# astojanov/Clover

Measured on AMD Instinct MI355X. Metric: int4 GEMV (CloverMatrix4::mvm) effective GB/s, algorithmic operand bytes / time, higher is better.
Workload: dtype int4; 1 GPU; CloverMatrix4::mvm 65536x65536 int4 (65536x65536 per GPU; preset c3: BASELINE configs[2] per GPU), x and result CloverVector4, STOCHASTIC_ROUNDING_DISABLED, bit-exact reference order; rows_per_gpu=65536, cols=65536, parallelism=row-shard x1, settle_launches=168

## Files before the change

clover_amd/csrc/matrix4.hip:

```cpp
#include "rng_device.h"

#include <stdlib.h>
#include <string.h>


#define MVM_CHUNK 65536u

template <int U, bool NT>
__device__ __forceinline__ void mvm_steps(const u32x4 *__restrict__ Ap, const u32x4 *xs, const float *cs, int q,
                                          uint32_t t0, float &a0, float &a1, float &a2, float &a3)
{
    u32x4 a[U];
#pragma unroll
    for (int u = 0; u < U; u++) a[u] = NT ? __builtin_nontemporal_load(&Ap[4 * (t0 + u) + q]) : Ap[4 * (t0 + u) + q];
#pragma unroll
    for (int u = 0; u < U; u++) {
        const u32x4 xv = xs[4 * (t0 + u) + q];
        const float c = cs[2 * (t0 + u) + (q >> 1)];
        a0 = __builtin_fmaf(c, (float)sdot8(a[u].x, xv.x, 0), a0);
        a1 = __builtin_fmaf(c, (float)sdot8(a[u].y, xv.y, 0), a1);
        a2 = __builtin_fmaf(c, (float)sdot8(a[u].z, xv.z, 0), a2);
        a3 = __builtin_fmaf(c, (float)sdot8(a[u].w, xv.w, 0), a3);
    }
}

template <int U, bool NT>
__device__ __forceinline__ void mvm_steps8(const u32x2 *__restrict__ Ap, const u32x2 *xs, const float *cs, int e, uint32_t t0, float &a0,
                                           float &a1)
{
    u32x2 a[U];
#pragma unroll
    for (int u = 0; u < U; u++) a[u] = NT ? __builtin_nontemporal_load(&Ap[8 * (t0 + u) + e]) : Ap[8 * (t0 + u) + e];
#pragma unroll
    for (int u = 0; u < U; u++) {
        const u32x2 xv = xs[8 * (t0 + u) + e];
        const float c = cs[2 * (t0 + u) + (e >> 2)];
        a0 = __builtin_fmaf(c, (float)sdot8(a[u].x, xv.x, 0), a0);
        a1 = __builtin_fmaf(c, (float)sdot8(a[u].y, xv.y, 0), a1);
    }
}

__device__ __forceinline__ int requantize_wave(float d, float noise, uint32_t *r_words, float *sr, float *scale)
{
    const int lane = threadIdx.x & 63;
    float m = wave_max(__builtin_fabsf(d));
    m = fix_zero_max(m);
    const float k = 7.0f / m;
    const int qv = quant1(d, k, noise);
    if (r_words) {
        uint32_t w = ((uint32_t)qv & 0xFu) << nib_shift(lane & 7);
        w |= __shfl_xor(w, 1);
        w |= __shfl_xor(w, 2);
        w |= __shfl_xor(w, 4);
        if ((lane & 7) == 0) r_words[lane >> 3] = w;
        if (lane == 0) *sr = m;
    }
    *scale = m;
    return qv;
}

struct MvmFuse {
    const uint32_t *qu;
    const float *su;
    float a;
    uint32_t *r2;
    float *sr2;
};

template <int U, bool NT, bool ST, bool FUSE, int L = 4>
__global__ __launch_bounds__(64 * L) void k_m4_mvm64(const uint8_t *__restrict__ A, const float *__restrict__ sA,
                                                  uint64_t cols, const uint8_t *__restrict__ x, const float *__restrict__ sx,
                                                  float *__restrict__ d_out, uint32_t *r, float *sr,
                                                  uint64_t *rng_state, uint64_t seq, const uint64_t *__restrict__ pow_rows, MvmFuse fuse)
{
    extern __shared__ __attribute__((aligned(16))) char smem[];
    u32x4 *xs = reinterpret_cast<u32x4 *>(smem);
    float *cs = reinterpret_cast<float *>(smem + MVM_CHUNK / 2);
    float *dsh = cs + MVM_CHUNK / 64;
    uint64_t *rbase = reinterpret_cast<uint64_t *>(dsh + 64);
    uint64_t *raw = rbase + 4;
    uint64_t *rbase2 = raw + 8, *raw2 = rbase2 + 4;
    if (ST) {
        const uint64_t a0 = rng_workgroup_begin(rng_state, seq, pow_rows, blockIdx.x, 1, (FUSE ? 4ull : 2ull) * gridDim.x, rbase);
        if (FUSE) {
            const uint64_t b2 = wave_pow_apply(pow_rows, a0, (uint64_t)gridDim.x + blockIdx.x, 1);
            if ((threadIdx.x & 63) == 0) rbase2[threadIdx.x >> 6] = b2;
        }
    }
    uint32_t fuse_w = 0;
    float fuse_s = 0.0f;
    if (FUSE && threadIdx.x < 64) {
        fuse_w = fuse.qu[blockIdx.x * 8 + (threadIdx.x >> 3)];
        fuse_s = fuse.su[blockIdx.x];
    }

    static_assert(L == 4 || (L == 8 && !ST), "the stochastic epilogue assumes 4 waves");
    constexpr int THREADS = 64 * L;
    const uint64_t rb = blockIdx.x;
    const int tid = threadIdx.x;
    const int q = tid & (L - 1);
    const int rho = tid / L;
    const uint64_t row = rb * 64 + rho;
    const u32x4 *Arow = reinterpret_cast<const u32x4 *>(A + row * (cols / 2));
    const float *sArow = sA + rb * (cols / 64);

    float a0 = 0.0f, a1 = 0.0f, a2 = 0.0f, a3 = 0.0f;

    for (uint64_t c0 = 0; c0 < cols; c0 += MVM_CHUNK) {
        const uint32_t cw = (uint32_t)((cols - c0) < MVM_CHUNK ? (cols - c0) : MVM_CHUNK);
        if (c0) __syncthreads();
        const u32x4 *xg = reinterpret_cast<const u32x4 *>(x + c0 / 2);
        {
            constexpr int NX = MVM_CHUNK / 32 / THREADS;
            constexpr int NC = MVM_CHUNK / 64 / THREADS;
            u32x4 xr[NX];
            float sa[NC], sv[NC];
            const uint32_t nx = cw / 32, nc = cw / 64;
#pragma unroll
            for (int k = 0; k < NX; k++) { const uint32_t i = tid + THREADS * k; xr[k] = xg[i < nx ? i : 0]; }
#pragma unroll
            for (int k = 0; k < NC; k++) {
                const uint32_t i = tid + THREADS * k, ii = i < nc ? i : 0;
                sa[k] = sArow[c0 / 64 + ii];
                sv[k] = sx[c0 / 64 + ii];
            }
#pragma unroll
            for (int k = 0; k < NX; k++) { const uint32_t i = tid + THREADS * k; if (i < nx) xs[i] = xr[k]; }
#pragma unroll
            for (int k = 0; k < NC; k++) { const uint32_t i = tid + THREADS * k; if (i < nc) cs[i] = (sa[k] * CLV_RCP49) * sv[k]; }
        }
        __syncthreads();

        const u32x4 *Ap = Arow + c0 / 32;
        const uint32_t npairs = cw / 128;
        uint32_t t = 0;
        if constexpr (L == 4) {
            for (; t + U <= npairs; t += U) mvm_steps<U, NT>(Ap, xs, cs, q, t, a0, a1, a2, a3);
            for (; t < npairs; t++) mvm_steps<1, NT>(Ap, xs, cs, q, t, a0, a1, a2, a3);
        } else {
            const u32x2 *Ap8 = reinterpret_cast<const u32x2 *>(Ap);
            const u32x2 *xs8 = reinterpret_cast<const u32x2 *>(xs);
            for (; t + U <= npairs; t += U) mvm_steps8<U, NT>(Ap8, xs8, cs, q, t, a0, a1);
            for (; t < npairs; t++) mvm_steps8<1, NT>(Ap8, xs8, cs, q, t, a0, a1);
        }
    }

    const float v0 = a0 + __shfl_xor(a0, 2);
    const float v1 = a1 + __shfl_xor(a1, 2);
    const float v2 = a2 + __shfl_xor(a2, 2);
    const float v3 = a3 + __shfl_xor(a3, 2);
    const float x0 = v0 + __shfl_xor(v0, 1);
    const float x1 = v1 + __shfl_xor(v1, 1);
    const float x2 = v2 + __shfl_xor(v2, 1);
    const float x3 = v3 + __shfl_xor(v3, 1);
    float dot = (x0 + x2) + (x1 + x3);
    if constexpr (L == 8) {
        const float u0 = a0 + __shfl_xor(a0, 4), u1 = a1 + __shfl_xor(a1, 4);
        const float y0 = u0 + __shfl_xor(u0, 2), y1 = u1 + __shfl_xor(u1, 2);
        const float z0 = y0 + __shfl_xor(y0, 1), z1 = y1 + __shfl_xor(y1, 1);
        dot = z0 + z1;
    }

    if (q == 0) {
        dsh[rho] = dot;
        if (d_out) d_out[row] = dot;
    }
    if (ST && tid < 4) {
        gen_blocks(rbase[tid], 1, raw, tid);
        if (FUSE) gen_blocks(rbase2[tid], 1, raw2, tid);
    }
    __syncthreads();
    if ((r || FUSE) && tid < 64) {
        float noise = 0.0f;
        if (ST) {
            const int grp = tid & 7, j = tid >> 3;
            noise = noise_of(reinterpret_cast<const uint32_t *>(raw + (size_t)(grp >> 2) * 4)[j], grp & 3);
        }
        float m;
        const int qv = requantize_wave(dsh[tid], noise, r ? r + rb * 8 : nullptr, r ? sr + rb : nullptr, &m);
        if (FUSE) {
            const float su7 = div7(fuse_s), sv7 = div7(m * fuse.a);
            const float val = __builtin_fmaf((float)qv, sv7, (float)unpack1(fuse_w, tid & 7) * su7);
            float noise2 = 0.0f;
            if (ST) {
                const int g = (tid & 7) ^ 1, j = tid >> 3;
                noise2 = noise_of(reinterpret_cast<const uint32_t *>(raw2 + (size_t)(g >> 2) * 4)[j], g & 3);
            }
            float m2;
            requantize_wave(val, noise2, fuse.r2 + rb * 8, fuse.sr2 + rb, &m2);
        }
    }
}

__global__ __launch_bounds__(256) void k_m4_quantize_strip(const float *__restrict__ A, uint64_t cols, uint32_t *__restrict__ q,
                                                           float *__restrict__ s, uint32_t strips_x, uint32_t tiles_x)
{
    __shared__ float sh[4][4];
    const uint32_t sj = blockIdx.x % strips_x;
    const uint64_t bi = blockIdx.x / strips_x;
    const int wave = threadIdx.x >> 6, lane = threadIdx.x & 63;
    const uint64_t col = (uint64_t)sj * 256 + 4 * lane;
    const bool live = col < cols;
    const uint64_t row0 = bi * 64 + wave * 16;

    f32x4 v[16];
    float m = 0.0f;
#pragma unroll
    for (int r = 0; r < 16; r++) {
        v[r] = live ? __builtin_nontemporal_load(reinterpret_cast<const f32x4 *>(A + (row0 + r) * cols + col)) : f32x4{0.0f, 0.0f, 0.0f, 0.0f};
        m = fmaxf(m, fmaxf(fmaxf(__builtin_fabsf(v[r].x), __builtin_fabsf(v[r].y)), fmaxf(__builtin_fabsf(v[r].z), __builtin_fabsf(v[r].w))));
    }
    m = row16_max(m);
    if ((lane & 15) == 0) sh[wave][lane >> 4] = m;
    __syncthreads();
    const int t = lane >> 4;
    m = fix_zero_max(fmaxf(fmaxf(sh[0][t], sh[1][t]), fmaxf(sh[2][t], sh[3][t])));
    const float k = 7.0f / m;
    if (wave == 0 && (lane & 15) == 0 && live) s[bi * tiles_x + sj * 4 + t] = m;
    const int odd = lane & 1;
#pragma unroll
    for (int r = 0; r < 16; r += 2) {
        const uint32_t h0 = quant_pack4(v[r], k), h1 = quant_pack4(v[r + 1], k);
        const uint32_t give = odd ? h0 : h1;
        const uint32_t recv = (uint32_t)__builtin_amdgcn_update_dpp(0, (int)give, 0xB1, 0xF, 0xF, false);
        const uint32_t word = odd ? (recv | (h1 << 16)) : (h0 | (recv << 16));
        if (live) __builtin_nontemporal_store(word, &q[((row0 + r + odd) * cols + (col & ~7ull)) / 8]);
    }
}

__global__ __launch_bounds__(256) void k_m4_gemm_simple(const uint8_t *__restrict__ A, const float *__restrict__ sA, uint64_t M,
                                                        uint64_t K, const uint8_t *__restrict__ B, const float *__restrict__ sB,
                                                        uint64_t N, float *__restrict__ C)
{
    const uint64_t j = (uint64_t)blockIdx.x * 16 + (threadIdx.x & 15);
    const uint64_t i = (uint64_t)blockIdx.y * 16 + (threadIdx.x >> 4);
    if (i >= M || j >= N) return;
    const uint64_t kb = K / 64;
    const u32x4 *a = reinterpret_cast<const u32x4 *>(A + i * (K / 2));
    const u32x4 *b = reinterpret_cast<const u32x4 *>(B + j * (K / 2));
    const float *sa = sA + (i >> 6) * kb;
    const float *sb = sB + (j >> 6) * kb;
    float acc = 0.0f;
    for (uint64_t blk = 0; blk < kb; blk++) {
        const int S = dot32(a[2 * blk], b[2 * blk]) + dot32(a[2 * blk + 1], b[2 * blk + 1]);
        const float c = (sa[blk] * CLV_RCP49) * sb[blk];
        acc = __builtin_fmaf(c, (float)S, acc);
    }
    C[i * N + j] = acc;
}

template <bool NT>
__global__ __launch_bounds__(256) void k_m4_restore(const uint32_t *__restrict__ q, const float *__restrict__ s, f32x4 *__restrict__ A,
                                                    uint64_t nquads, uint64_t cols)
{
    const uint64_t f0 = ((uint64_t)blockIdx.x * 4 + (threadIdx.x >> 6)) * 256;
    const int lane = threadIdx.x & 63;
    const uint64_t tiles_x = cols / 64;
    uint32_t wd[4];
    float sc[4];
#pragma unroll
    for (int j = 0; j < 4; j++) {
        const uint64_t f = f0 + 64 * j + lane, fc = f < nquads ? f : 0;
        const uint64_t e = fc * 4, row = e / cols, col = e - row * cols;
        wd[j] = q[fc >> 1];
        sc[j] = s[(row >> 6) * tiles_x + (col >> 6)];
    }
#pragma unroll
    for (int j = 0; j < 4; j++) {
        const uint64_t f = f0 + 64 * j + lane;
        const uint32_t hw = wd[j] >> (16 * (lane & 1));
        const float k = div7(sc[j]);
        f32x4 v;
        v.x = (float)(((int)(hw << 24)) >> 28) * k;
        v.y = (float)(((int)(hw << 28)) >> 28) * k;
        v.z = (float)(((int)(hw << 16)) >> 28) * k;
        v.w = (float)(((int)(hw << 20)) >> 28) * k;
        if (f < nquads) {
            if (NT) __builtin_nontemporal_store(v, &A[f]);
            else A[f] = v;
        }
    }
}

int clm4_quantize_stochastic(const float *A, uint64_t rows, uint64_t cols, int8_t *q, float *s, uint64_t *rng, hipStream_t st);
int clm4_gemm_mfma(const int8_t *A, const float *sA, uint64_t M, uint64_t K, const int8_t *B, const float *sB, uint64_t N, float *C, hipStream_t st);
int clm4_gemm_fp6(const int8_t *A, const float *sA, uint64_t M, uint64_t K, const int8_t *B, const float *sB, uint64_t N, float *C, hipStream_t st);

#define MVM_LDS_BYTES (MVM_CHUNK / 2 + (MVM_CHUNK / 64) * sizeof(float) + 64 * sizeof(float) + 256)

static int launch_mvm(const int8_t *A, const float *sA, uint64_t rows, uint64_t cols, const int8_t *x, const float *sx,
                      float *d, int8_t *r, float *sr, uint64_t *rng, hipStream_t st, const MvmFuse *fuse = nullptr)
{
    const size_t lds = MVM_LDS_BYTES;
    const dim3 grid((unsigned)(rows / 64)), block(256);
    RngTables T = {nullptr, nullptr, nullptr};
    uint64_t seq = 0;
    if (rng) {
        int rc = clv_rng_tables(&T);
        if (rc) return rc;
        seq = clv_rng_seq_for(rng, st);
    }
    const MvmFuse no_fuse = {nullptr, nullptr, 0.0f, nullptr, nullptr};
#define MVM_LAUNCH_F(NT, ST, FUSE)                                                                                               \
    hipLaunchKernelGGL((k_m4_mvm64<8, NT, ST, FUSE>), grid, block, lds, st, (const uint8_t *)A, sA, cols, (const uint8_t *)x, sx, d, \
                       (uint32_t *)r, sr, rng, seq, T.pow_rows, FUSE ? *fuse : no_fuse)
#define MVM_LAUNCH(NT, ST)                                  \
    do {                                                    \
        if (fuse) MVM_LAUNCH_F(NT, ST, true);               \
        else MVM_LAUNCH_F(NT, ST, false);                   \
    } while (0)
    const bool streaming = rows * (cols / 2) > (256ull << 20);
    const bool wide = streaming && !rng && rows / 64 <= 2ull * (uint64_t)clv_cu_count();
    if (wide) {
        if (fuse)
            hipLaunchKernelGGL((k_m4_mvm64<16, true, false, true, 8>), grid, dim3(512), lds, st, (const uint8_t *)A, sA, cols,
                               (const uint8_t *)x, sx, d, (uint32_t *)r, sr, rng, seq, T.pow_rows, *fuse);
        else
            hipLaunchKernelGGL((k_m4_mvm64<16, true, false, false, 8>), grid, dim3(512), lds, st, (const uint8_t *)A, sA, cols,
                               (const uint8_t *)x, sx, d, (uint32_t *)r, sr, rng, seq, T.pow_rows, no_fuse);
    } else if (streaming) {
        if (rng) MVM_LAUNCH(true, true); else MVM_LAUNCH(true, false);
    } else {
        if (rng) MVM_LAUNCH(false, true); else MVM_LAUNCH(false, false);
    }
#undef MVM_LAUNCH
#undef MVM_LAUNCH_F
    CLV_LAUNCH_CHECK();
    return CLV_OK;
}

#ifdef CLV_EXPERIMENTS
__global__ __launch_bounds__(256) void k_read_bw(const u32x4 *__restrict__ p, uint64_t n16, uint32_t *__restrict__ out, int nt)
{
    const uint64_t stride = (uint64_t)gridDim.x * blockDim.x;
    uint32_t acc = 0;
    uint64_t i = (uint64_t)blockIdx.x * blockDim.x + threadIdx.x;
    for (; i + 7 * stride < n16; i += 8 * stride) {
        u32x4 v[8];
#pragma unroll
        for (int u = 0; u < 8; u++) v[u] = nt ? __builtin_nontemporal_load(&p[i + u * stride]) : p[i + u * stride];
#pragma unroll
        for (int u = 0; u < 8; u++) acc ^= v[u].x ^ v[u].y ^ v[u].z ^ v[u].w;
    }
    for (; i < n16; i += stride) { const u32x4 v = p[i]; acc ^= v.x ^ v.y ^ v.z ^ v.w; }
    if (acc == 0x12345678u) out[0] = acc;
}

extern "C" int clvx_read_bw(const void *p, uint64_t bytes, int nt, int blocks_per_cu, void *out, void *stream)
{
    hipLaunchKernelGGL(k_read_bw, dim3(clv_cu_count() * blocks_per_cu), dim3(256), 0, as_stream(stream), (const u32x4 *)p, bytes / 16,
                       (uint32_t *)out, nt);
    CLV_LAUNCH_CHECK();
    return CLV_OK;
}

extern "C" int clvx_mvm_variant(int variant, const int8_t *A, const float *sA, uint64_t rows, uint64_t cols, const int8_t *x,
                                const float *sx, int8_t *r, float *sr, void *stream)
{
    const size_t lds = MVM_LDS_BYTES;
    hipStream_t st = as_stream(stream);
    const dim3 grid((unsigned)(rows / 64)), block(256);
#define CLVX_LAUNCH(U, NT)                                                                                                      \
    hipLaunchKernelGGL((k_m4_mvm64<U, NT, false, false>), grid, block, lds, st, (const uint8_t *)A, sA, cols, (const uint8_t *)x, sx, \
                       (float *)nullptr, (uint32_t *)r, sr, (uint64_t *)nullptr, 0ull, (const uint64_t *)nullptr,                      \
                       MvmFuse{nullptr, nullptr, 0.0f, nullptr, nullptr})
    switch (variant) {
    case 0: CLVX_LAUNCH(8, true); break;
    case 1: CLVX_LAUNCH(8, false); break;
    case 2: CLVX_LAUNCH(4, true); break;
    case 3: CLVX_LAUNCH(16, true); break;
    case 4: CLVX_LAUNCH(2, true); break;
    case 5: CLVX_LAUNCH(16, false); break;
    case 6: CLVX_LAUNCH(32, false); break;
#define CLVX_LAUNCH8(U, NT)                                                                                                       \
    hipLaunchKernelGGL((k_m4_mvm64<U, NT, false, false, 8>), grid, dim3(512), lds, st, (const uint8_t *)A, sA, cols, (const uint8_t *)x, \
                       sx, (float *)nullptr, (uint32_t *)r, sr, (uint64_t *)nullptr, 0ull, (const uint64_t *)nullptr,                 \
                       MvmFuse{nullptr, nullptr, 0.0f, nullptr, nullptr})
    case 7: CLVX_LAUNCH8(8, false); break;
    case 8: CLVX_LAUNCH8(16, false); break;
    case 9: CLVX_LAUNCH8(8, true); break;
    case 10: CLVX_LAUNCH8(16, true); break;
#undef CLVX_LAUNCH8
    default: clv_set_error("clvx_mvm_variant: unknown variant %d", variant); return CLV_ERR_INVALID;
    }
#undef CLVX_LAUNCH
    CLV_LAUNCH_CHECK();
    return CLV_OK;
}
#endif

static int check_mvm_args(const char *fn, const void *A, const void *sA, uint64_t rows, uint64_t cols, const void *x, const void *sx)
{
    CLV_REQUIRE(A && sA && x && sx, "%s: null pointer", fn);
    CLV_REQUIRE(rows % 64 == 0 && cols % 128 == 0, "%s: rows=%llu must be a multiple of 64 and cols=%llu of 128", fn,
                (unsigned long long)rows, (unsigned long long)cols);
    CLV_REQUIRE(rows / 64 <= 0x7FFFFFFFull, "%s: too many rows", fn);
    return CLV_OK;
}

extern "C" int clm4_restore(const int8_t *q, const float *s, uint64_t rows, uint64_t cols, float *A, void *stream)
{
    CLV_REQUIRE(A && q && s, "clm4_restore: null pointer");
    CLV_REQUIRE(rows % 128 == 0 && cols % 128 == 0, "clm4_restore: rows=%llu cols=%llu must be multiples of 128", (unsigned long long)rows,
                (unsigned long long)cols);
    if (!rows || !cols) return CLV_OK;
    const uint64_t nquads = rows * cols / 4, waves = (nquads + 255) / 256;
    CLV_REQUIRE((waves + 3) / 4 <= 0x7FFFFFFFull, "clm4_restore: matrix too large");
    if (rows * cols * sizeof(float) > (256ull << 20))
        hipLaunchKernelGGL(k_m4_restore<true>, dim3((unsigned)((waves + 3) / 4)), dim3(256), 0, as_stream(stream), (const uint32_t *)q, s,
                           (f32x4 *)A, nquads, cols);
    else
        hipLaunchKernelGGL(k_m4_restore<false>, dim3((unsigned)((waves + 3) / 4)), dim3(256), 0, as_stream(stream), (const uint32_t *)q, s,
                           (f32x4 *)A, nquads, cols);
    CLV_LAUNCH_CHECK();
    return CLV_OK;
}

extern "C" int clm4_mvm(const int8_t *A, const float *sA, uint64_t rows, uint64_t cols, const int8_t *x, const float *sx,
                        int8_t *r, float *sr, uint64_t *rng_state_dev, void *stream)
{
    int rc = check_mvm_args("clm4_mvm", A, sA, rows, cols, x, sx);
    if (rc) return rc;
    CLV_REQUIRE(r && sr, "clm4_mvm: null result pointer");
    if (!rows) return CLV_OK;
    hipStream_t st = as_stream(stream);
    return launch_mvm(A, sA, rows, cols, x, sx, nullptr, r, sr, rng_state_dev, st);
}

extern "C" int clm4_mvm_scale_and_add(const int8_t *A, const float *sA, uint64_t rows, uint64_t cols, const int8_t *x, const float *sx,
                                      const int8_t *qu, const float *su, float a, int8_t *t, float *st_, int8_t *r, float *sr,
                                      uint64_t *rng_state_dev, void *stream)
{
    int rc = check_mvm_args("clm4_mvm_scale_and_add", A, sA, rows, cols, x, sx);
    if (rc) return rc;
    CLV_REQUIRE(qu && su && r && sr, "clm4_mvm_scale_and_add: null pointer");
    CLV_REQUIRE((t == nullptr) == (st_ == nullptr), "clm4_mvm_scale_and_add: t and st must both be given or both be NULL");
    CLV_REQUIRE((const void *)r != (const void *)x && (const void *)sr != (const void *)sx,
                "clm4_mvm_scale_and_add: the result must not alias the vector being multiplied");
    if (!rows) return CLV_OK;
    const MvmFuse fuse = {(const uint32_t *)qu, su, a, (uint32_t *)r, sr};
    return launch_mvm(A, sA, rows, cols, x, sx, nullptr, t, st_, rng_state_dev, as_stream(stream), &fuse);
}

extern "C" int clm4_rowdots(const int8_t *A, const float *sA, uint64_t rows, uint64_t cols, const int8_t *x, const float *sx,
                            float *d, void *stream)
{
    int rc = check_mvm_args("clm4_rowdots", A, sA, rows, cols, x, sx);
    if (rc) return rc;
    CLV_REQUIRE(d, "clm4_rowdots: null result pointer");
    if (!rows) return CLV_OK;
    return launch_mvm(A, sA, rows, cols, x, sx, d, nullptr, nullptr, nullptr, as_stream(stream));
}

extern "C" int clm4_quantize(const float *A, uint64_t rows, uint64_t cols, int8_t *q, float *s, uint64_t *rng_state_dev, void *stream)
{
    CLV_REQUIRE(A && q && s, "clm4_quantize: null pointer");
    CLV_REQUIRE(rows % 128 == 0 && cols % 128 == 0, "clm4_quantize: rows=%llu cols=%llu must be multiples of 128",
                (unsigned long long)rows, (unsigned long long)cols);
    if (!rows || !cols) return CLV_OK;
    const uint64_t tiles = (rows / 64) * (cols / 64);
    CLV_REQUIRE(tiles <= 0x7FFFFFFFull, "clm4_quantize: too many tiles");
    if (rng_state_dev) return clm4_quantize_stochastic(A, rows, cols, q, s, rng_state_dev, as_stream(stream));
    const uint32_t strips_x = (uint32_t)((cols + 255) / 256);
    hipLaunchKernelGGL(k_m4_quantize_strip, dim3((unsigned)((rows / 64) * strips_x)), dim3(256), 0, as_stream(stream), A, cols,
                       (uint32_t *)q, s, strips_x, (uint32_t)(cols / 64));
    CLV_LAUNCH_CHECK();
    return CLV_OK;
}

extern "C" int clm4_gemm(const int8_t *A, const float *sA, uint64_t M, uint64_t K, const int8_t *B, const float *sB, uint64_t N,
                         float *C, void *stream)
{
    CLV_REQUIRE(A && sA && B && sB && C, "clm4_gemm: null pointer");
    CLV_REQUIRE(M % 128 == 0 && N % 128 == 0 && K % 128 == 0, "clm4_gemm: M=%llu N=%llu K=%llu must be multiples of 128",
                (unsigned long long)M, (unsigned long long)N, (unsigned long long)K);
    if (!M || !N) return CLV_OK;
    static const int which = [] { const char *e = clv_env("CLV_GEMM_KERNEL"); return !e ? 0 : !strcmp(e, "simple") ? 2 : !strcmp(e, "i8") ? 1 : 0; }();
    if (which == 0 && K > 0) return clm4_gemm_fp6(A, sA, M, K, B, sB, N, C, as_stream(stream));
    if (which == 1 && K > 0) return clm4_gemm_mfma(A, sA, M, K, B, sB, N, C, as_stream(stream));
    hipLaunchKernelGGL(k_m4_gemm_simple, dim3((unsigned)(N / 16), (unsigned)(M / 16)), dim3(256), 0, as_stream(stream),
                       (const uint8_t *)A, sA, M, K, (const uint8_t *)B, sB, N, C);
    CLV_LAUNCH_CHECK();
    return CLV_OK;
}
```

clover_amd/lib_binding.py:

```python
from __future__ import annotations

import ctypes as C
from pathlib import Path

import numpy as np

from .build import hip_library_path

DOT_EXACT = 0
DOT_FAST = 1
THRESHOLD_FAST = 0
THRESHOLD_REFERENCE = 1

_vp = C.c_void_p
_u64 = C.c_uint64

SIGNATURES = {
    "clv_version": (C.c_char_p, []),
    "clv_last_error": (C.c_char_p, []),
    "clv_device_count": (C.c_int, [C.POINTER(C.c_int)]),
    "clv_set_device": (C.c_int, [C.c_int]),
    "clv_get_device": (C.c_int, [C.POINTER(C.c_int)]),
    "clv_device_info": (C.c_int, [C.c_char_p, C.c_int, C.POINTER(C.c_int), C.POINTER(_u64)]),
    "clv_malloc": (C.c_int, [C.POINTER(_vp), _u64]),
    "clv_free": (C.c_int, [_vp]),
    "clv_memset": (C.c_int, [_vp, C.c_int, _u64, _vp]),
    "clv_memcpy_h2d": (C.c_int, [_vp, _vp, _u64, _vp]),
    "clv_memcpy_d2h": (C.c_int, [_vp, _vp, _u64, _vp]),
    "clv_memcpy_d2d": (C.c_int, [_vp, _vp, _u64, _vp]),
    "clv_host_alloc": (C.c_int, [C.POINTER(_vp), _u64]),
    "clv_host_free": (C.c_int, [_vp]),
    "clv_stream_create": (C.c_int, [C.POINTER(_vp)]),
    "clv_stream_destroy": (C.c_int, [_vp]),
    "clv_stream_sync": (C.c_int, [_vp]),
    "clv_device_sync": (C.c_int, []),
    "clv_event_create": (C.c_int, [C.POINTER(_vp)]),
    "clv_event_destroy": (C.c_int, [_vp]),
    "clv_event_record": (C.c_int, [_vp, _vp]),
    "clv_event_sync": (C.c_int, [_vp]),
    "clv_event_elapsed_ms": (C.c_int, [_vp, _vp, C.POINTER(C.c_float)]),
    "clv_rng_seed": (C.c_int, [_vp, _u64, _u64, _vp]),
    "clv_rng_set": (C.c_int, [_vp, C.POINTER(_u64), C.POINTER(_u64), _vp]),
    "clv_rng_get": (C.c_int, [_vp, C.POINTER(_u64), C.POINTER(_u64), _vp]),
    "clv_rng_graph_mode": (C.c_int, [_vp, C.c_int, _vp]),
    "clv_rng_set_segments": (C.c_int, [C.c_int]),
    "clv4_quantize": (C.c_int, [_vp, _u64, _vp, _vp, _vp, _vp]),
    "clv4_restore": (C.c_int, [_vp, _vp, _u64, _vp, _vp]),
    "clv4_dot_workspace_bytes": (_u64, [_u64]),
    "clv4_dot": (C.c_int, [_vp, _vp, _vp, _vp, _u64, C.c_int, _vp, _vp, _vp]),
    "clv8_dot_workspace_bytes": (_u64, [_u64]),
    "clv8_dot": (C.c_int, [_vp, _vp, _vp, _vp, _u64, C.c_int, _vp, _vp, _vp]),
    "clv4_word_isums": (C.c_int, [_vp, _vp, _u64, _vp, _vp]),
    "clm4_quantize": (C.c_int, [_vp, _u64, _u64, _vp, _vp, _vp, _vp]),
    "clm4_restore": (C.c_int, [_vp, _vp, _u64, _u64, _vp, _vp]),
    "clm4_mvm": (C.c_int, [_vp, _vp, _u64, _u64, _vp, _vp, _vp, _vp, _vp, _vp]),
    "clm4_rowdots": (C.c_int, [_vp, _vp, _u64, _u64, _vp, _vp, _vp, _vp]),
    "clm4_gemm": (C.c_int, [_vp, _vp, _u64, _u64, _vp, _vp, _u64, _vp, _vp]),
    "clm4_gemm_prepare": (C.c_int, [_vp, _u64, _u64, C.POINTER(_vp), _vp]),
    "clm4_gemm_release": (C.c_int, [_vp]),
    "clm4_gemm_prepared": (C.c_int, [_vp, _vp, _vp, _u64, _u64, _vp, _vp, _vp, _u64, _vp, _vp]),
    "clm4_gemm_i32": (C.c_int, [_vp, _u64, _u64, _vp, _u64, _u64, _u64, _vp, _vp]),
    "clm4_gemm_i32_prepared": (C.c_int, [_vp, _vp, _u64, _u64, _vp, _vp, _u64, _u64, _u64, _vp, _vp]),
    "clv4_scale_and_add": (C.c_int, [_vp, _vp, _vp, _vp, C.c_float, _u64, _vp, _vp, _vp, _vp]),
    "clm4_mvm_scale_and_add": (C.c_int, [_vp, _vp, _u64, _u64, _vp, _vp, _vp, _vp, C.c_float, _vp, _vp, _vp, _vp, _vp, _vp]),
    "clv8_quantize": (C.c_int, [_vp, _u64, _vp, _vp, _vp, _vp]),
    "clv8_restore": (C.c_int, [_vp, _vp, _u64, _vp, _vp]),
    "clv8_scale_and_add": (C.c_int, [_vp, _vp, _vp, _vp, C.c_float, _u64, _vp, _vp, _vp, _vp]),
    "clv8_threshold_workspace_bytes": (_u64, [_u64]),
    "clv8_threshold": (C.c_int, [_vp, _vp, _u64, _u64, _u64, _vp, _vp]),
    "clv8_threshold_mode": (C.c_int, [_vp, _vp, _u64, _u64, _u64, C.c_int, _vp, _vp]),
    "clm4_mvm_v8": (C.c_int, [_vp, _vp, _u64, _u64, _vp, _vp, _vp, _vp, _vp, _vp]),
    "clm4_mvm_v8_scale_and_add": (C.c_int, [_vp, _vp, _u64, _u64, _vp, _vp, _vp, _vp, C.c_float, _vp, _vp, _vp, _vp, _vp, _vp]),
    "clv_iht_persistent_launches": (_u64, []),
    "clm4_iht_v8": (C.c_int, [_vp, _vp, _vp, _vp, _u64, _u64, _vp, _vp, _u64, _vp, _vp, _vp, _vp, _vp, _vp, _vp, _vp, _u64, _u64, C.c_float,
                              C.c_int, _vp, _vp]),
    "clm4_rowdots_v8": (C.c_int, [_vp, _vp, _u64, _u64, _vp, _vp, _vp, _vp]),
    "clv4_threshold_workspace_bytes": (_u64, [_u64]),
    "clv4_threshold": (C.c_int, [_vp, _vp, _u64, _u64, _u64, _vp, _vp]),
    "clv_threshold_reference_workspace_bytes": (_u64, [_u64]),
    "clv_threshold_reference_workspace_bytes_k": (_u64, [_u64, _u64]),
    "clv4_threshold_mode": (C.c_int, [_vp, _vp, _u64, _u64, _u64, C.c_int, _vp, _vp]),
    "clv4_threshold_heap": (C.c_int, [_vp, _vp, _u64, _u64, _u64, _vp, _vp, _vp]),
    "clv8_threshold_heap": (C.c_int, [_vp, _vp, _u64, _u64, _u64, _vp, _vp, _vp]),
    "clm4_transpose": (C.c_int, [_vp, _vp, _u64, _u64, _vp, _vp, _vp]),
    "clm4_mvm_f32": (C.c_int, [_vp, _vp, _u64, _u64, _vp, _vp, _vp]),
    "clm8_quantize": (C.c_int, [_vp, _u64, _u64, _vp, _vp, _vp, _vp]),
    "clm8_restore": (C.c_int, [_vp, _vp, _u64, _u64, _vp, _vp]),
    "clm8_mvm": (C.c_int, [_vp, _vp, _u64, _u64, _vp, _vp, _vp, _vp, _vp, _vp]),
    "clm8_mvm_f32": (C.c_int, [_vp, _vp, _u64, _u64, _vp, _vp, _vp]),
    "clm8_transpose": (C.c_int, [_vp, _vp, _u64, _u64, _vp, _vp, _vp]),
    "clv_f16_quantize": (C.c_int, [_vp, _u64, _vp, _vp]),
    "clv_f16_restore": (C.c_int, [_vp, _u64, _vp, _vp]),
    "clv_f16_scale_and_add": (C.c_int, [_vp, _vp, C.c_float, _u64, _vp, _vp]),
    "clv_f16_dot_workspace_bytes": (_u64, [_u64]),
    "clv_f16_dot": (C.c_int, [_vp, _vp, _u64, C.c_int, _vp, _vp, _vp]),
    "clv_f16_threshold_workspace_bytes": (_u64, [_u64]),
    "clv_f16_threshold_mode": (C.c_int, [_vp, _u64, _u64, _u64, C.c_int, _vp, _vp]),
    "clv_f16_threshold_heap": (C.c_int, [_vp, _u64, _u64, _u64, _vp, _vp, _vp]),
    "clm_f16_quantize": (C.c_int, [_vp, _u64, _u64, _vp, _vp]),
    "clm_f16_mvm": (C.c_int, [_vp, _u64, _u64, _vp, _vp, _vp]),
    "clm_f16_mvm_f32": (C.c_int, [_vp, _u64, _u64, _vp, _vp, _vp]),
    "clm_f16_transpose": (C.c_int, [_vp, _u64, _u64, _vp, _vp]),
    "clm4_iht": (C.c_int, [_vp, _vp, _vp, _vp, _u64, _u64, _vp, _vp, _u64, _vp, _vp, _vp, _vp, _vp, _vp, _vp, _vp, _u64, _u64,
                          C.c_float, C.c_int, _vp, _vp]),
    "clm4_shard_partition": (C.c_int, [_u64, C.c_int, C.c_int, C.POINTER(_u64), C.POINTER(_u64)]),
    "clm4_sharded_create": (C.c_int, [C.POINTER(_vp), C.c_int, C.POINTER(C.c_int), _u64, _u64]),
    "clm4_sharded_destroy": (C.c_int, [_vp]),
    "clm4_sharded_info": (C.c_int, [_vp, C.c_int, C.POINTER(C.c_int), C.POINTER(_u64), C.POINTER(_u64), C.POINTER(_vp), C.POINTER(_vp)]),
# ... 390 lines not shown
```

include/clover_hip.h:

```cpp
#ifndef CLOVER_HIP_H
#define CLOVER_HIP_H

#include <stdint.h>

#ifdef __cplusplus
extern "C" {
#endif

#define CLV_OK                 0
#define CLV_ERR_INVALID       -1
#define CLV_ERR_HIP           -2
#define CLV_ERR_NO_DEVICE     -3
#define CLV_ERR_UNSUPPORTED   -4

#define CLV_DOT_EXACT          0
#define CLV_DOT_FAST           1

const char *clv_version(void);
const char *clv_last_error(void);
int  clv_device_count(int *count);
int  clv_set_device(int device);
int  clv_get_device(int *device);
int  clv_device_info(char *name, int name_len, int *compute_units, uint64_t *hbm_bytes);

int  clv_malloc(void **ptr, uint64_t bytes);
int  clv_free(void *ptr);
int  clv_memset(void *ptr, int value, uint64_t bytes, void *stream);
int  clv_memcpy_h2d(void *dst_dev, const void *src_host, uint64_t bytes, void *stream);
int  clv_memcpy_d2h(void *dst_host, const void *src_dev, uint64_t bytes, void *stream);
int  clv_memcpy_d2d(void *dst_dev, const void *src_dev, uint64_t bytes, void *stream);
int  clv_host_alloc(void **ptr, uint64_t bytes);
int  clv_host_free(void *ptr);
int  clv_stream_create(void **stream);
int  clv_stream_destroy(void *stream);
int  clv_stream_sync(void *stream);
int  clv_device_sync(void);
int  clv_event_create(void **event);
int  clv_event_destroy(void *event);
int  clv_event_record(void *event, void *stream);
int  clv_event_sync(void *event);
int  clv_event_elapsed_ms(void *start, void *stop, float *ms);

#define CLV_RNG_STATE_BYTES 256
int  clv_rng_seed(uint64_t *state_dev, uint64_t key1, uint64_t key2, void *stream);
int  clv_rng_set(uint64_t *state_dev, const uint64_t key1[4], const uint64_t key2[4], void *stream);
int  clv_rng_get(const uint64_t *state_dev, uint64_t key1[4], uint64_t key2[4], void *stream);
int  clv_rng_graph_mode(uint64_t *state_dev, int on, void *stream);
int  clv_rng_set_segments(int segments);

int  clv4_quantize(const float *x, uint64_t n_pad, int8_t *q, float *s, uint64_t *rng_state_dev, void *stream);
int  clv4_restore(const int8_t *q, const float *s, uint64_t n_pad, float *x, void *stream);
uint64_t clv4_dot_workspace_bytes(uint64_t n_pad);
int  clv4_dot(const int8_t *qu, const float *su, const int8_t *qv, const float *sv, uint64_t n_pad,
              int mode, float *out_dev, void *workspace, void *stream);
int  clv4_word_isums(const int8_t *qu, const int8_t *qv, uint64_t n_pad, int32_t *isums, void *stream);

int  clm4_quantize(const float *A, uint64_t rows, uint64_t cols, int8_t *q, float *s,
                   uint64_t *rng_state_dev, void *stream);
int  clm4_restore(const int8_t *q, const float *s, uint64_t rows, uint64_t cols, float *A, void *stream);
int  clm4_mvm(const int8_t *A, const float *sA, uint64_t rows, uint64_t cols,
              const int8_t *x, const float *sx, int8_t *r, float *sr,
              uint64_t *rng_state_dev, void *stream);
int  clm4_rowdots(const int8_t *A, const float *sA, uint64_t rows, uint64_t cols,
                  const int8_t *x, const float *sx, float *d, void *stream);
int  clm4_gemm(const int8_t *A, const float *sA, uint64_t M, uint64_t K,
               const int8_t *B, const float *sB, uint64_t N, float *C, void *stream);

typedef struct clm4_gemm_operand clm4_gemm_operand;
int  clm4_gemm_prepare(const int8_t *q, uint64_t rows, uint64_t K, clm4_gemm_operand **op, void *stream);
int  clm4_gemm_release(clm4_gemm_operand *op);
int  clm4_gemm_prepared(const clm4_gemm_operand *opA, const int8_t *A, const float *sA, uint64_t M, uint64_t K,
                        const clm4_gemm_operand *opB, const int8_t *B, const float *sB, uint64_t N, float *C, void *stream);
int  clm4_gemm_i32(const int8_t *A, uint64_t M, uint64_t K, const int8_t *B, uint64_t N, uint64_t kb_begin, uint64_t kb_count,
                   int32_t *S, void *stream);
int  clm4_gemm_i32_prepared(const clm4_gemm_operand *opA, const int8_t *A, uint64_t M, uint64_t K,
                            const clm4_gemm_operand *opB, const int8_t *B, uint64_t N, uint64_t kb_begin, uint64_t kb_count,
                            int32_t *S, void *stream);

int  clv4_scale_and_add(const int8_t *qu, const float *su, const int8_t *qv, const float *sv, float a, uint64_t n_pad,
                        int8_t *r, float *sr, uint64_t *rng_state_dev, void *stream);
int  clm4_mvm_scale_and_add(const int8_t *A, const float *sA, uint64_t rows, uint64_t cols, const int8_t *x, const float *sx,
                            const int8_t *qu, const float *su, float a, int8_t *t, float *st, int8_t *r, float *sr,
                            uint64_t *rng_state_dev, void *stream);
int  clv8_quantize(const float *x, uint64_t n_pad, int8_t *q, float *s, uint64_t *rng_state_dev, void *stream);
int  clv8_restore(const int8_t *q, const float *s, uint64_t n_pad, float *x, void *stream);
int  clv8_scale_and_add(const int8_t *qu, const float *su, const int8_t *qv, const float *sv, float a, uint64_t n_pad,
                        int8_t *r, float *sr, uint64_t *rng_state_dev, void *stream);
uint64_t clv8_dot_workspace_bytes(uint64_t n_pad);
int  clv8_dot(const int8_t *qu, const float *su, const int8_t *qv, const float *sv, uint64_t n_pad, int mode, float *out_dev,
              void *workspace, void *stream);
uint64_t clv8_threshold_workspace_bytes(uint64_t n_pad);
int  clv8_threshold(int8_t *q, const float *s, uint64_t n, uint64_t n_pad, uint64_t k, void *workspace, void *stream);
int  clv8_threshold_mode(int8_t *q, const float *s, uint64_t n, uint64_t n_pad, uint64_t k, int mode, void *workspace, void *stream);
int  clm4_mvm_v8(const int8_t *A, const float *sA, uint64_t rows, uint64_t cols, const int8_t *x, const float *sx,
                 int8_t *r, float *sr, uint64_t *rng_state_dev, void *stream);
int  clm4_mvm_v8_scale_and_add(const int8_t *A, const float *sA, uint64_t rows, uint64_t cols, const int8_t *x, const float *sx,
                               const int8_t *qu, const float *su, float a, int8_t *t, float *st, int8_t *r, float *sr,
                               uint64_t *rng_state_dev, void *stream);
int  clm4_iht_v8(const int8_t *Phi, const float *sPhi, const int8_t *PhiT, const float *sPhiT, uint64_t m, uint64_t n,
                 int8_t *x, float *sx, uint64_t x_len, const int8_t *y, const float *sy, int8_t *t1, float *st1,
                 int8_t *t2, float *st2, int8_t *t3, float *st3, uint64_t iterations, uint64_t K, float mu, int threshold,
                 uint64_t *rng_state_dev, void *stream);
uint64_t clv_iht_persistent_launches(void);
int  clm4_rowdots_v8(const int8_t *A, const float *sA, uint64_t rows, uint64_t cols, const int8_t *x, const float *sx,
                     float *d, void *stream);
uint64_t clv4_threshold_workspace_bytes(uint64_t n_pad);
int  clv4_threshold(int8_t *q, const float *s, uint64_t n, uint64_t n_pad, uint64_t k, void *workspace, void *stream);
#define CLV_THRESHOLD_FAST 0
#define CLV_THRESHOLD_REFERENCE 1
uint64_t clv_threshold_reference_workspace_bytes(uint64_t n_pad);
uint64_t clv_threshold_reference_workspace_bytes_k(uint64_t n_pad, uint64_t k);
int  clv4_threshold_mode(int8_t *q, const float *s, uint64_t n, uint64_t n_pad, uint64_t k, int mode, void *workspace, void *stream);
int  clv4_threshold_heap(int8_t *q, const float *s, uint64_t n, uint64_t n_pad, uint64_t k, void *heap_dev, void *workspace, void *stream);
int  clv8_threshold_heap(int8_t *q, const float *s, uint64_t n, uint64_t n_pad, uint64_t k, void *heap_dev, void *workspace, void *stream);
int  clm4_transpose(const int8_t *q, const float *s, uint64_t rows, uint64_t cols, int8_t *qt, float *st, void *stream);
// ... 64 lines not shown
```

Measured before the change: 6542 GB/s.

## Group two row blocks per workgroup sharing one staged x chunk in LDS

Adds a grouped MVM kernel path in which each workgroup processes G row blocks (default 2, 512 threads) and shares a single LDS copy of the x chunk, with per-group scale buffers. The first A loads of each chunk are also issued before the LDS stores and barrier, so they overlap x staging. For large deterministic matrices with between 4 and 8 row blocks per CU, this is meant to cut redundant x staging and per-workgroup startup latency. In exchange the launch bounds rise and occupancy changes, and debug timestamp probes are threaded through behind a probe macro.

New measurement: 6716 GB/s (median of 6 runs). 1.03x the previous value.

```diff
diff --git a/clover_amd/csrc/matrix4.hip b/clover_amd/csrc/matrix4.hip
--- a/clover_amd/csrc/matrix4.hip
+++ b/clover_amd/csrc/matrix4.hip
@@ -5,6 +5,8 @@
 
 
 #define MVM_CHUNK 65536u
+#define MVM_GROUP_RULE 2
+#define MVM_GROUP_MAX_PER_CU 8ull
 
 template <int U, bool NT>
 __device__ __forceinline__ void mvm_steps(const u32x4 *__restrict__ Ap, const u32x4 *xs, const float *cs, int q,
@@ -13,6 +15,28 @@
     u32x4 a[U];
 #pragma unroll
     for (int u = 0; u < U; u++) a[u] = NT ? __builtin_nontemporal_load(&Ap[4 * (t0 + u) + q]) : Ap[4 * (t0 + u) + q];
+#pragma unroll
+    for (int u = 0; u < U; u++) {
+        const u32x4 xv = xs[4 * (t0 + u) + q];
+        const float c = cs[2 * (t0 + u) + (q >> 1)];
+        a0 = __builtin_fmaf(c, (float)sdot8(a[u].x, xv.x, 0), a0);
+        a1 = __builtin_fmaf(c, (float)sdot8(a[u].y, xv.y, 0), a1);
+        a2 = __builtin_fmaf(c, (float)sdot8(a[u].z, xv.z, 0), a2);
+        a3 = __builtin_fmaf(c, (float)sdot8(a[u].w, xv.w, 0), a3);
+    }
+}
+
+template <int U, bool NT>
+__device__ __forceinline__ void mvm_request(const u32x4 *__restrict__ Ap, int q, uint32_t t0, u32x4 (&a)[U])
+{
+#pragma unroll
+    for (int u = 0; u < U; u++) a[u] = NT ? __builtin_nontemporal_load(&Ap[4 * (t0 + u) + q]) : Ap[4 * (t0 + u) + q];
+}
+
+template <int U>
+__device__ __forceinline__ void mvm_consume(const u32x4 (&a)[U], const u32x4 *xs, const float *cs, int q, uint32_t t0, float &a0,
+                                            float &a1, float &a2, float &a3)
+{
 #pragma unroll
     for (int u = 0; u < U; u++) {
         const u32x4 xv = xs[4 * (t0 + u) + q];
@@ -67,12 +91,131 @@
     float *sr2;
 };
 
-template <int U, bool NT, bool ST, bool FUSE, int L = 4>
-__global__ __launch_bounds__(64 * L) void k_m4_mvm64(const uint8_t *__restrict__ A, const float *__restrict__ sA,
+#define MVM_G_STAMP(i) CLV_PROBE(do { if (dbg && threadIdx.x == 0) dbg[blockIdx.x * 8 + (i)] = __builtin_amdgcn_s_memrealtime(); } while (0))
+
+template <int U, bool NT, int G, bool FIRST, bool HEAD>
+__device__ __forceinline__ void mvm_grouped_chunk(const u32x4 *__restrict__ Ap, const float *__restrict__ sAp, uint32_t cw,
+                                                  const u32x4 *__restrict__ xg, const float *__restrict__ sxp, u32x4 *xs, float *cs,
+                                                  int tid, int lt, int q, float &a0, float &a1, float &a2,
+                                                  float &a3 CLV_PROBE(, unsigned long long *dbg))
+{
+    constexpr int THREADS = 256 * G;
+    constexpr int NX = MVM_CHUNK / 32 / THREADS;
+    constexpr int NC = MVM_CHUNK / 64 / 256;
+    const uint32_t nx = cw / 32, nc = cw / 64, npairs = cw / 128;
+    if (!FIRST) __syncthreads();
+    u32x4 xr[NX];
+    float sa[NC], sv[NC];
+#pragma unroll
+    for (int k = 0; k < NX; k++) { const uint32_t i = tid + THREADS * k; xr[k] = xg[i < nx ? i : 0]; }
+#pragma unroll
+    for (int k = 0; k < NC; k++) {
+        const uint32_t i = lt + 256 * k, ii = i < nc ? i : 0;
+        sa[k] = sAp[ii];
+        sv[k] = sxp[ii];
+    }
+    u32x4 a[U];
+    if constexpr (HEAD) mvm_request<U, NT>(Ap, q, 0, a);
+#pragma unroll
+    for (int k = 0; k < NX; k++) xs[tid + THREADS * k] = xr[k];
+#pragma unroll
+    for (int k = 0; k < NC; k++) cs[lt + 256 * k] = (sa[k] * CLV_RCP49) * sv[k];
+    __syncthreads();
+    CLV_PROBE(if (FIRST) MVM_G_STAMP(1);)
+    if constexpr (HEAD) {
+        mvm_consume<U>(a, xs, cs, q, 0, a0, a1, a2, a3);
+        CLV_PROBE(if (FIRST) MVM_G_STAMP(2);)
+        for (uint32_t t = U; t + U <= npairs; t += U) mvm_steps<U, NT>(Ap, xs, cs, q, t, a0, a1, a2, a3);
+    }
+    for (uint32_t t = npairs / U * U; t < npairs; t++) mvm_steps<1, NT>(Ap, xs, cs, q, t, a0, a1, a2, a3);
+}
+
+template <int U, bool NT, int G, bool FIRST>
+__device__ __forceinline__ void mvm_grouped_chunk_at(const u32x4 *__restrict__ Arow, const float *__restrict__ sArow, uint64_t cols,
+                                                     uint64_t c0, const uint8_t *__restrict__ x, const float *__restrict__ sx, u32x4 *xs,
+                                                     float *cs, int tid, int lt, int q, float &a0, float &a1, float &a2,
+                                                     float &a3 CLV_PROBE(, unsigned long long *dbg))
+{
+    const uint32_t cw = (uint32_t)((cols - c0) < MVM_CHUNK ? (cols - c0) : MVM_CHUNK);
+    const u32x4 *xg = reinterpret_cast<const u32x4 *>(x + c0 / 2);
+    if (cw / 128 >= (uint32_t)U)
+        mvm_grouped_chunk<U, NT, G, FIRST, true>(Arow + c0 / 32, sArow + c0 / 64, cw, xg, sx + c0 / 64, xs, cs, tid, lt, q, a0, a1, a2, a3 CLV_PROBE(, dbg));
+    else
+        mvm_grouped_chunk<U, NT, G, FIRST, false>(Arow + c0 / 32, sArow + c0 / 64, cw, xg, sx + c0 / 64, xs, cs, tid, lt, q, a0, a1, a2, a3 CLV_PROBE(, dbg));
+}
+
+template <int U, bool NT, bool FUSE, int G>
+__device__ __forceinline__ void mvm64_grouped(const uint8_t *__restrict__ A, const float *__restrict__ sA, uint64_t cols,
+                                              const uint8_t *__restrict__ x, const float *__restrict__ sx, float *__restrict__ d_out,
+                                              uint32_t *r, float *sr, const MvmFuse &fuse, uint32_t nrb CLV_PROBE(, unsigned long long *dbg))
+{
+    extern __shared__ __attribute__((aligned(16))) char smem[];
+    u32x4 *xs = reinterpret_cast<u32x4 *>(smem);
+    const int tid = threadIdx.x;
+    const int g = tid >> 8, lt = tid & 255;
+    float *cs = reinterpret_cast<float *>(smem + MVM_CHUNK / 2) + g * (MVM_CHUNK / 64);
+    float *dsh = reinterpret_cast<float *>(smem + MVM_CHUNK / 2) + G * (MVM_CHUNK / 64) + g * 64;
+    MVM_G_STAMP(0);
+
+    const uint64_t rb_own = (uint64_t)blockIdx.x * G + g;
+    const bool present = rb_own < nrb;
+    const uint64_t rb = present ? rb_own : nrb - 1;
+    uint32_t fuse_w = 0;
+    float fuse_s = 0.0f;
+    if (FUSE && lt < 64) {
+        fuse_w = fuse.qu[rb * 8 + (lt >> 3)];
+        fuse_s = fuse.su[rb];
+    }
+    const int q = lt & 3, rho = lt >> 2;
+    const uint64_t row = rb * 64 + rho;
+    const u32x4 *Arow = reinterpret_cast<const u32x4 *>(A + row * (cols / 2));
+    const float *sArow = sA + rb * (cols / 64);
+
+    float a0 = 0.0f, a1 = 0.0f, a2 = 0.0f, a3 = 0.0f;
+    mvm_grouped_chunk_at<U, NT, G, true>(Arow, sArow, cols, 0, x, sx, xs, cs, tid, lt, q, a0, a1, a2, a3 CLV_PROBE(, dbg));
+    for (uint64_t c0 = MVM_CHUNK; c0 < cols; c0 += MVM_CHUNK)
+        mvm_grouped_chunk_at<U, NT, G, false>(Arow, sArow, cols, c0, x, sx, xs, cs, tid, lt, q, a0, a1, a2, a3 CLV_PROBE(, dbg));
+    MVM_G_STAMP(3);
+
+    const float v0 = a0 + __shfl_xor(a0, 2);
+    const float v1 = a1 + __shfl_xor(a1, 2);
+    const float v2 = a2 + __shfl_xor(a2, 2);
+    const float v3 = a3 + __shfl_xor(a3, 2);
+    const float x0 = v0 + __shfl_xor(v0, 1);
+    const float x1 = v1 + __shfl_xor(v1, 1);
+    const float x2 = v2 + __shfl_xor(v2, 1);
+    const float x3 = v3 + __shfl_xor(v3, 1);
+    const float dot = (x0 + x2) + (x1 + x3);
+    if (q == 0) {
+        dsh[rho] = dot;
+        if (d_out && present) d_out[row] = dot;
+    }
+    __syncthreads();
+    if ((r || FUSE) && lt < 64 && present) {
+        float m;
+        const int qv = requantize_wave(dsh[lt], 0.0f, r ? r + rb * 8 : nullptr, r ? sr + rb : nullptr, &m);
+        if (FUSE) {
+            const float su7 = div7(fuse_s), sv7 = div7(m * fuse.a);
+            const float val = __builtin_fmaf((float)qv, sv7, (float)unpack1(fuse_w, lt & 7) * su7);
+            float m2;
+            requantize_wave(val, 0.0f, fuse.r2 + rb * 8, fuse.sr2 + rb, &m2);
+        }
+    }
+    MVM_G_STAMP(4);
+}
+
+template <int U, bool NT, bool ST, bool FUSE, int L = 4, int G = 1>
+__global__ __launch_bounds__(64 * L * G, G == 2 ? 4 : 1) void k_m4_mvm64(const uint8_t *__restrict__ A, const float *__restrict__ sA,
                                                   uint64_t cols, const uint8_t *__restrict__ x, const float *__restrict__ sx,
                                                   float *__restrict__ d_out, uint32_t *r, float *sr,
-                                                  uint64_t *rng_state, uint64_t seq, const uint64_t *__restrict__ pow_rows, MvmFuse fuse)
-{
+                                                  uint64_t *rng_state, uint64_t seq, const uint64_t *__restrict__ pow_rows, MvmFuse fuse,
+                                                  uint32_t nrb CLV_PROBE(, unsigned long long *dbg))
+{
+    static_assert(G == 1 || (L == 4 && !ST), "row blocks are grouped on the 4-lanes-per-row deterministic kernel only");
+    if constexpr (G > 1) {
+        mvm64_grouped<U, NT, FUSE, G>(A, sA, cols, x, sx, d_out, r, sr, fuse, nrb CLV_PROBE(, dbg));
+        return;
+    }
     extern __shared__ __attribute__((aligned(16))) char smem[];
     u32x4 *xs = reinterpret_cast<u32x4 *>(smem);
     float *cs = reinterpret_cast<float *>(smem + MVM_CHUNK / 2);
@@ -95,6 +238,7 @@
     }
 
     static_assert(L == 4 || (L == 8 && !ST), "the stochastic epilogue assumes 4 waves");
+    MVM_G_STAMP(0);
     constexpr int THREADS = 64 * L;
     const uint64_t rb = blockIdx.x;
     const int tid = threadIdx.x;
@@ -130,12 +274,16 @@
             for (int k = 0; k < NC; k++) { const uint32_t i = tid + THREADS * k; if (i < nc) cs[i] = (sa[k] * CLV_RCP49) * sv[k]; }
         }
         __syncthreads();
+        CLV_PROBE(if (!c0) MVM_G_STAMP(1);)
 
         const u32x4 *Ap = Arow + c0 / 32;
         const uint32_t npairs = cw / 128;
         uint32_t t = 0;
         if constexpr (L == 4) {
-            for (; t + U <= npairs; t += U) mvm_steps<U, NT>(Ap, xs, cs, q, t, a0, a1, a2, a3);
+            for (; t + U <= npairs; t += U) {
+                mvm_steps<U, NT>(Ap, xs, cs, q, t, a0, a1, a2, a3);
+                CLV_PROBE(if (!c0 && !t) MVM_G_STAMP(2);)
+            }
             for (; t < npairs; t++) mvm_steps<1, NT>(Ap, xs, cs, q, t, a0, a1, a2, a3);
         } else {
             const u32x2 *Ap8 = reinterpret_cast<const u32x2 *>(Ap);
@@ -145,6 +293,7 @@
         }
     }
 
+    MVM_G_STAMP(3);
     const float v0 = a0 + __shfl_xor(a0, 2);
     const float v1 = a1 + __shfl_xor(a1, 2);
     const float v2 = a2 + __shfl_xor(a2, 2);
@@ -190,6 +339,7 @@
             requantize_wave(val, noise2, fuse.r2 + rb * 8, fuse.sr2 + rb, &m2);
         }
     }
+    MVM_G_STAMP(4);
 }
 
 __global__ __launch_bounds__(256) void k_m4_quantize_strip(const float *__restrict__ A, uint64_t cols, uint32_t *__restrict__ q,
@@ -287,12 +437,41 @@
 int clm4_gemm_fp6(const int8_t *A, const float *sA, uint64_t M, uint64_t K, const int8_t *B, const float *sB, uint64_t N, float *C, hipStream_t st);
 
 #define MVM_LDS_BYTES (MVM_CHUNK / 2 + (MVM_CHUNK / 64) * sizeof(float) + 64 * sizeof(float) + 256)
+#define MVM_LDS_BYTES_G(G) (MVM_CHUNK / 2 + (G) * ((MVM_CHUNK / 64) * sizeof(float) + 64 * sizeof(float)))
+
+template <int G>
+static void launch_mvm_grouped(const int8_t *A, const float *sA, uint64_t rows, uint64_t cols, const int8_t *x, const float *sx, float *d,
+                               int8_t *r, float *sr, bool nt, hipStream_t st, const MvmFuse *fuse CLV_PROBE(, unsigned long long *dbg = nullptr))
+{
+    const uint32_t nrb = (uint32_t)(rows / 64);
+    const dim3 grid((nrb + G - 1) / G), block(256 * G);
+    const size_t lds = MVM_LDS_BYTES_G(G);
+    const MvmFuse no_fuse = {nullptr, nullptr, 0.0f, nullptr, nullptr};
+#define MVM_LAUNCH_G(NT, FUSE)                                                                                                         \
+    hipLaunchKernelGGL((k_m4_mvm64<8, NT, false, FUSE, 4, G>), grid, block, lds, st, (const uint8_t *)A, sA, cols, (const uint8_t *)x, sx, \
+                       d, (uint32_t *)r, sr, (uint64_t *)nullptr, 0ull, (const uint64_t *)nullptr, FUSE ? *fuse : no_fuse,               \
+                       nrb CLV_PROBE(, dbg))
+    if (nt) { if (fuse) MVM_LAUNCH_G(true, true); else MVM_LAUNCH_G(true, false); }
+    else { if (fuse) MVM_LAUNCH_G(false, true); else MVM_LAUNCH_G(false, false); }
+#undef MVM_LAUNCH_G
+}
+
+static int mvm_group_for(uint64_t rows, uint64_t cols, bool stochastic)
+{
+    if (stochastic || !cols) return 1;
+    const int forced = (int)clv_env_int("CLV_MVM_GROUP", 0);
+    if (forced == 1 || forced == 2 || forced == 4) return forced;
+    const bool streaming = rows * (cols / 2) > (256ull << 20);
+    const uint64_t nrb = rows / 64, cus = (uint64_t)clv_cu_count();
+    return streaming && nrb >= 4 * cus && nrb <= MVM_GROUP_MAX_PER_CU * cus ? MVM_GROUP_RULE : 1;
+}
 
 static int launch_mvm(const int8_t *A, const float *sA, uint64_t rows, uint64_t cols, const int8_t *x, const float *sx,
                       float *d, int8_t *r, float *sr, uint64_t *rng, hipStream_t st, const MvmFuse *fuse = nullptr)
 {
     const size_t lds = MVM_LDS_BYTES;
     const dim3 grid((unsigned)(rows / 64)), block(256);
+    const uint32_t nrb = (uint32_t)(rows / 64);
     RngTables T = {nullptr, nullptr, nullptr};
     uint64_t seq = 0;
     if (rng) {
@@ -303,7 +482,7 @@
     const MvmFuse no_fuse = {nullptr, nullptr, 0.0f, nullptr, nullptr};
 #define MVM_LAUNCH_F(NT, ST, FUSE)                                                                                               \
     hipLaunchKernelGGL((k_m4_mvm64<8, NT, ST, FUSE>), grid, block, lds, st, (const uint8_t *)A, sA, cols, (const uint8_t *)x, sx, d, \
-                       (uint32_t *)r, sr, rng, seq, T.pow_rows, FUSE ? *fuse : no_fuse)
+                       (uint32_t *)r, sr, rng, seq, T.pow_rows, FUSE ? *fuse : no_fuse, nrb CLV_PROBE(, (unsigned long long *)nullptr))
 #define MVM_LAUNCH(NT, ST)                                  \
     do {                                                    \
         if (fuse) MVM_LAUNCH_F(NT, ST, true);               \
@@ -311,13 +490,16 @@
     } while (0)
     const bool streaming = rows * (cols / 2) > (256ull << 20);
     const bool wide = streaming && !rng && rows / 64 <= 2ull * (uint64_t)clv_cu_count();
-    if (wide) {
+    const int group = mvm_group_for(rows, cols, rng != nullptr);
+    if (group == 4) launch_mvm_grouped<4>(A, sA, rows, cols, x, sx, d, r, sr, streaming, st, fuse);
+    else if (group == 2) launch_mvm_grouped<2>(A, sA, rows, cols, x, sx, d, r, sr, streaming, st, fuse);
+    else if (wide) {
         if (fuse)
             hipLaunchKernelGGL((k_m4_mvm64<16, true, false, true, 8>), grid, dim3(512), lds, st, (const uint8_t *)A, sA, cols,
-                               (const uint8_t *)x, sx, d, (uint32_t *)r, sr, rng, seq, T.pow_rows, *fuse);
+                               (const uint8_t *)x, sx, d, (uint32_t *)r, sr, rng, seq, T.pow_rows, *fuse, nrb CLV_PROBE(, (unsigned long long *)nullptr));
         else
             hipLaunchKernelGGL((k_m4_mvm64<16, true, false, false, 8>), grid, dim3(512), lds, st, (const uint8_t *)A, sA, cols,
-                               (const uint8_t *)x, sx, d, (uint32_t *)r, sr, rng, seq, T.pow_rows, no_fuse);
+                               (const uint8_t *)x, sx, d, (uint32_t *)r, sr, rng, seq, T.pow_rows, no_fuse, nrb CLV_PROBE(, (unsigned long long *)nullptr));
     } else if (streaming) {
         if (rng) MVM_LAUNCH(true, true); else MVM_LAUNCH(true, false);
     } else {
@@ -354,16 +536,18 @@
     return CLV_OK;
 }
 
-extern "C" int clvx_mvm_variant(int variant, const int8_t *A, const float *sA, uint64_t rows, uint64_t cols, const int8_t *x,
-                                const float *sx, int8_t *r, float *sr, void *stream)
+extern "C" int clvx_mvm_variant_stamped(int variant, const int8_t *A, const float *sA, uint64_t rows, uint64_t cols, const int8_t *x,
+                                        const float *sx, int8_t *r, float *sr, void *stamps, void *stream)
 {
     const size_t lds = MVM_LDS_BYTES;
     hipStream_t st = as_stream(stream);
     const dim3 grid((unsigned)(rows / 64)), block(256);
+    unsigned long long *dbg = (unsigned long long *)stamps;
+    CLV_REQUIRE(!dbg || variant == 0 || variant == 11 || variant == 12, "clvx_mvm_variant_stamped: variant %d writes no stamps", variant);
 #define CLVX_LAUNCH(U, NT)                                                                                                      \
     hipLaunchKernelGGL((k_m4_mvm64<U, NT, false, false>), grid, block, lds, st, (const uint8_t *)A, sA, cols, (const uint8_t *)x, sx, \
                        (float *)nullptr, (uint32_t *)r, sr, (uint64_t *)nullptr, 0ull, (const uint64_t *)nullptr,                      \
-                       MvmFuse{nullptr, nullptr, 0.0f, nullptr, nullptr})
+                       MvmFuse{nullptr, nullptr, 0.0f, nullptr, nullptr}, (uint32_t)(rows / 64), dbg)
     switch (variant) {
     case 0: CLVX_LAUNCH(8, true); break;
     case 1: CLVX_LAUNCH(8, false); break;
@@ -375,17 +559,25 @@
 #define CLVX_LAUNCH8(U, NT)                                                                                                       \
     hipLaunchKernelGGL((k_m4_mvm64<U, NT, false, false, 8>), grid, dim3(512), lds, st, (const uint8_t *)A, sA, cols, (const uint8_t *)x, \
                        sx, (float *)nullptr, (uint32_t *)r, sr, (uint64_t *)nullptr, 0ull, (const uint64_t *)nullptr,                 \
-                       MvmFuse{nullptr, nullptr, 0.0f, nullptr, nullptr})
+                       MvmFuse{nullptr, nullptr, 0.0f, nullptr, nullptr}, (uint32_t)(rows / 64), dbg)
     case 7: CLVX_LAUNCH8(8, false); break;
     case 8: CLVX_LAUNCH8(16, false); break;
     case 9: CLVX_LAUNCH8(8, true); break;
     case 10: CLVX_LAUNCH8(16, true); break;
 #undef CLVX_LAUNCH8
+    case 11: launch_mvm_grouped<4>(A, sA, rows, cols, x, sx, nullptr, r, sr, true, st, nullptr, dbg); break;
+    case 12: launch_mvm_grouped<2>(A, sA, rows, cols, x, sx, nullptr, r, sr, true, st, nullptr, dbg); break;
     default: clv_set_error("clvx_mvm_variant: unknown variant %d", variant); return CLV_ERR_INVALID;
     }
 #undef CLVX_LAUNCH
     CLV_LAUNCH_CHECK();
     return CLV_OK;
+}
+
+extern "C" int clvx_mvm_variant(int variant, const int8_t *A, const float *sA, uint64_t rows, uint64_t cols, const int8_t *x,
+                                const float *sx, int8_t *r, float *sr, void *stream)
+{
+    return clvx_mvm_variant_stamped(variant, A, sA, rows, cols, x, sx, r, sr, nullptr, stream);
 }
 #endif
 
@@ -442,6 +634,11 @@
     return launch_mvm(A, sA, rows, cols, x, sx, nullptr, t, st_, rng_state_dev, as_stream(stream), &fuse);
 }
 
+extern "C" int clm4_mvm_row_blocks_per_workgroup(uint64_t rows, uint64_t cols, int stochastic)
+{
+    return mvm_group_for(rows, cols, stochastic != 0);
+}
+
 extern "C" int clm4_rowdots(const int8_t *A, const float *sA, uint64_t rows, uint64_t cols, const int8_t *x, const float *sx,
                             float *d, void *stream)
 {
diff --git a/clover_amd/lib_binding.py b/clover_amd/lib_binding.py
--- a/clover_amd/lib_binding.py
+++ b/clover_amd/lib_binding.py
@@ -54,6 +54,7 @@
     "clm4_quantize": (C.c_int, [_vp, _u64, _u64, _vp, _vp, _vp, _vp]),
     "clm4_restore": (C.c_int, [_vp, _vp, _u64, _u64, _vp, _vp]),
     "clm4_mvm": (C.c_int, [_vp, _vp, _u64, _u64, _vp, _vp, _vp, _vp, _vp, _vp]),
+    "clm4_mvm_row_blocks_per_workgroup": (C.c_int, [_u64, _u64, C.c_int]),
     "clm4_rowdots": (C.c_int, [_vp, _vp, _u64, _u64, _vp, _vp, _vp, _vp]),
     "clm4_gemm": (C.c_int, [_vp, _vp, _u64, _u64, _vp, _vp, _u64, _vp, _vp]),
     "clm4_gemm_prepare": (C.c_int, [_vp, _u64, _u64, C.POINTER(_vp), _vp]),
diff --git a/include/clover_hip.h b/include/clover_hip.h
--- a/include/clover_hip.h
+++ b/include/clover_hip.h
@@ -61,6 +61,7 @@
 int  clm4_mvm(const int8_t *A, const float *sA, uint64_t rows, uint64_t cols,
               const int8_t *x, const float *sx, int8_t *r, float *sr,
               uint64_t *rng_state_dev, void *stream);
+int  clm4_mvm_row_blocks_per_workgroup(uint64_t rows, uint64_t cols, int stochastic);
 int  clm4_rowdots(const int8_t *A, const float *sA, uint64_t rows, uint64_t cols,
                   const int8_t *x, const float *sx, float *d, void *stream);
 int  clm4_gemm(const int8_t *A, const float *sA, uint64_t M, uint64_t K,
```
